# HBioquant/DiffBindFR

Hardware: AMD Instinct MI355X
Metric: poses_per_sec (higher is better)
Workload: dtype f32

## Files before the change

diffbindfr_amd/csrc/api.cpp:

```cpp
#include <cmath>
#include <cstdio>
#include <cstring>
#include <algorithm>
#include <atomic>
#include <map>

#include "launch.h"
#include "pack.h"

static unsigned long long convz_sc_lanes(const ConvZ& z) {
  unsigned long long m = 0;
  for (int i = 0; i < z.n_io; ++i) m |= 0xfffull << (z.out_off[i] / 4);
  return m;
}
static inline double fused_bytes(int D_in, int D_out) { return 4.0 * (48 + 9 + 3 + 48 + 48 + D_in + D_out); }

#define RT_TABLE static const
#include "residue_tables.inc"
#undef RT_TABLE

static thread_local std::string g_err;
void dbfr_set_error(const std::string& s) { g_err = s; }
static int fail(int code, const std::string& s) { g_err = s; return code; }

// ... 28 lines not shown
  if (!strcmp(e, "f32") || !strcmp(e, "0")) return DBFR_GEMM_F32;
  if (!strcmp(e, "split_f16") || !strcmp(e, "3")) return DBFR_GEMM_SPLIT_F16;
  if (!strcmp(e, "reduce_first") || !strcmp(e, "4")) return DBFR_GEMM_REDUCE_FIRST;
  return -1;
}

struct dbfr_model {
  dbfr_model_cfg cfg;
  std::vector<void*> allocs;
  ConvW layer[8][4];
  ConvW final_conv, tor_conv, sc_conv;
  ConvW2 layer2[8][4], tor_conv2, sc_conv2;
  ConvW2 layer2v[8][4];
  ConvZ layerz[8][4], tor_convz, sc_convz;
  int use_conv2;
  int gemm_split;
  int* queue;
  std::string fallback_convs;
  std::string rowscaled_convs;
  uint32_t layer_fallback;
  int* edge_log; int edge_log_steps, edge_log_graphs;
  int* tie_log; int tie_log_steps, tie_log_graphs; float tie_tol;
  Mlp2 lig_node_emb, lig_edge_emb, atom_edge_emb, la_edge_emb, center_edge_emb, tor_edge_emb, sc_edge_emb;
  Mlp2 tr_final, rot_final, tor_final, sc_final;
  const float* atom_emb[5]; int atom_dims[5];
  const float* atom_lin_t;
  const float *gs_lig_off, *gs_lig_c, *gs_atom_off, *gs_atom_c, *gs_cross_off, *gs_cross_c, *gs_center_off, *gs_center_c;
  int* a14_group;
  int profile;
  std::vector<hipEvent_t> ev;
// ... 182 lines not shown
      cfg->sigma_embed_dim != EMB || cfg->num_conv_layers < 1 || cfg->num_conv_layers > 8)
    return fail(DBFR_ERR_ARG, "unsupported model configuration (need ns=48, nv=12, sh_lmax=2, 32-d embeddings)");
  if (cfg->lig_edge_features + 2 * EMB > 80 || cfg->lig_node_features + EMB > 80)
    return fail(DBFR_ERR_ARG, "ligand feature width too large");
  std::string serr;
  int rc = so3_selftest(serr);
  if (rc) return fail(rc, serr);
  TMap tm;
  for (int i = 0; i < n_tensors; ++i) tm[tensors[i].name] = &tensors[i];
  dbfr_model* m = new dbfr_model();
  m->cfg = *cfg;
  m->profile = 0; m->ev_used = 0; m->flops_dev = nullptr; m->fused_bytes_last = 0; m->executed_last = 0; m->useful_last = 0; m->form_bytes_last = 0; m->conv_ms_acc = 0; m->conv_launches_acc = 0;
  m->edge_log = nullptr; m->edge_log_steps = 0; m->edge_log_graphs = 0; m->layer_fallback = 0;
  m->tie_log = nullptr; m->tie_log_steps = 0; m->tie_log_graphs = 0; m->tie_tol = 0.f;
  m->use_conv2 = getenv("DBFR_CONV2") ? atoi(getenv("DBFR_CONV2")) : -1;
  m->gemm_split = gemm_from_env();
  if (m->gemm_split < 0) rc = fail(DBFR_ERR_ARG, std::string("DBFR_GEMM=") + getenv("DBFR_GEMM") + ": unknown or retired value (f32 | split_f16 | reduce_first)");
  const char* fam[4] = {"lig_conv_layers", "cross_al_conv_layers", "atom_conv_layers", "cross_la_conv_layers"};
  for (int l = 0; l < cfg->num_conv_layers && !rc; ++l)
    for (int f = 0; f < 4 && !rc; ++f)
      rc = pack_conv144(m, tm, std::string(fam[f]) + "." + std::to_string(l), std::min(l, 3), &m->layer[l][f], &m->layer2[l][f], &m->layer2v[l][f], &m->layerz[l][f], 1u << l);
  ConvTensors final_t;
  if (!rc) rc = conv_tensors(tm, "final_conv", 4, &final_t);
  if (!rc) rc = pack_upload<PackedConv>(m, &m->final_conv, [&](PackedConv* p) { return pack_conv(final_t, 4, "final_conv", p); });
  if (!rc) rc = pack_conv144(m, tm, "tor_bond_conv", 5, &m->tor_conv, &m->tor_conv2, nullptr, &m->tor_convz, 1u << 31);
  if (!rc && !cfg->no_sc_torsion) rc = pack_conv144(m, tm, "sc_tor_bond_conv", 5, &m->sc_conv, &m->sc_conv2, nullptr, &m->sc_convz, 1u << 31);
  if (!rc) rc = pack_mlp(m, tm, "lig_node_embedding", cfg->lig_node_features + EMB, NS, NS, true, &m->lig_node_emb);
  if (!rc) rc = pack_mlp(m, tm, "lig_edge_embedding", cfg->lig_edge_features + 2 * EMB, NS, NS, true, &m->lig_edge_emb);
  if (!rc) rc = pack_mlp(m, tm, "atom_edge_embedding", 2 * EMB, NS, NS, true, &m->atom_edge_emb);
  if (!rc) rc = pack_mlp(m, tm, "la_edge_embedding", 2 * EMB, NS, NS, true, &m->la_edge_emb);
// ... 181 lines not shown
  s.chunk_es = S.chunk_es; s.chunk_gl = S.chunk_gl; s.n_chunks = S.chunk0 + G; s.max_chunks = S.chunk_cap; s.xmax = xmax; s.chunk_segs = chunk_segs;
  return s;
}

static ConvArgs conv_args(const ConvSite& s, const ConvW& cw) {
  ConvArgs a;
  a.n_edges = s.n_edges; a.max_edges = s.max_edges; a.tgt = s.tgt; a.gth = s.gth; a.emb = s.emb; a.sh = s.sh; a.sh_sign = 1.f;
  a.tab1 = s.tab1; a.ld1 = s.ld1; a.idx1 = s.idx1; a.tab2 = s.tab2; a.ld2 = s.ld2; a.idx2 = s.idx2; a.x = s.x; a.ldx = s.ldx;
  a.w = cw; a.msg = s.msg; a.trace = nullptr;
  return a;
}

static Conv2Desc conv2_desc(const ConvSite& s, const ConvW2& cw) {
  Conv2Desc d;
  d.n_edges = s.n_edges; d.max_edges = s.max_edges; d.gth = s.gth; d.emb = s.emb; d.sh = s.sh; d.tab1 = s.tab1; d.ld1 = s.ld1; d.idx1 = s.idx1;
  d.tab2 = s.tab2; d.ld2 = s.ld2; d.idx2 = s.idx2; d.x = s.x; d.ldx = s.ldx; d.w = cw; d.msg = s.msg;
  return d;
}

static ConvZDesc convz_desc(const ConvSite& s, const ConvZ& z, int D_out) {
  ConvZDesc o;
  o.n_edges = s.n_edges; o.max_edges = s.max_edges; o.tgt = s.tgt; o.gth = s.gth; o.emb = s.emb; o.sh = s.sh;
  o.tab1 = s.tab1; o.ld1 = s.ld1; o.idx1 = s.idx1; o.tab2 = s.tab2; o.ld2 = s.ld2; o.idx2 = s.idx2; o.x = s.x; o.ldx = s.ldx;
  o.w = z; o.msg = s.msg; o.D_out = D_out; o.chunk_es = s.chunk_es; o.chunk_gl = s.chunk_gl; o.n_chunks = s.n_chunks; o.max_chunks = s.max_chunks; o.xmax = s.xmax;
  return o;
}

static void conv_call(dbfr_model* m, const ConvW& cw, const ConvSite& site, hipStream_t st) {
  const ConvArgs a = conv_args(site, cw);
  hipEvent_t e0 = nullptr, e1 = nullptr;
  const bool prof = m->profile == 1 && cw.K == 144;
  const bool count = m->profile && cw.K == 144;
  if (prof) {
    prof_events(m, &e0, &e1);
    (void)hipEventRecord(e0, st);
  }
  launch_conv(a, st);
  if (prof) (void)hipEventRecord(e1, st);
  if (count) {
    launch_acc_flops(a.n_edges, 2.0 * cw.K * ((double)cw.K + cw.W), 4.0 * (cw.W + cw.D_in + 9) + 16.0, fused_bytes(cw.D_in, cw.D_out), m->flops_dev, st);
  }
}

static void conv2_call(dbfr_model* m, const Conv2Desc* descs, const int* Ws, int n, hipStream_t st, bool f16_fallback = false, const ConvZDesc* z = nullptr,
                       const int64_t* const* zsegs = nullptr) {
  Conv2Args a;
  memset(&a, 0, sizeof a);
  for (int i = 0; i < n; ++i) a.c[i] = descs[i];
  a.n_conv = n; a.queue = m->queue;
  hipEvent_t e0 = nullptr, e1 = nullptr;
  if (m->profile == 1) {
    prof_events(m, &e0, &e1);
    (void)hipEventRecord(e0, st);
  }
  static unsigned long long* trace_dev = nullptr;
  static const char* trace_file = getenv("DBFR_CONV2_TRACE");
  if (trace_file && !trace_dev) {
    if (hipMalloc(&trace_dev, 8 * C2_TRACE_CAP * sizeof(unsigned long long)) != hipSuccess) trace_dev = nullptr;
    else atexit([] {
      std::vector<unsigned long long> h(8 * C2_TRACE_CAP);
      if (hipDeviceSynchronize() == hipSuccess && hipMemcpy(h.data(), trace_dev, h.size() * 8, hipMemcpyDeviceToHost) == hipSuccess) {
        if (FILE* f = fopen(getenv("DBFR_CONV2_TRACE"), "wb")) { fwrite(h.data(), 8, h.size(), f); fclose(f); }
      }
    });
  }
  if (trace_dev) { (void)hipMemsetAsync(trace_dev, 0, 8 * C2_TRACE_CAP * sizeof(unsigned long long), st); a.trace = trace_dev; }
  if (z) {
    Conv2Args v = a;
    v.n_conv = 0;
    for (int i = 0; i < n; ++i)
      if (descs[i].w.n_tiles > 0) v.c[v.n_conv++] = descs[i];
    if (v.n_conv) launch_conv2h(v, st);
    ConvZArgs za;
    memset(&za, 0, sizeof za);
    for (int i = 0; i < n; ++i) za.c[i] = z[i];
    za.n_conv = n;
    za.dbg = nullptr;
    za.executed = m->profile ? m->flops_dev + 3 : nullptr;
    launch_convz(za, st, !zsegs);
  }
  else if (m->gemm_split >= DBFR_GEMM_SPLIT_F16 && !f16_fallback) launch_conv2h(a, st);
  else launch_conv2(a, st);
  if (m->profile == 1) (void)hipEventRecord(e1, st);
  if (m->profile) {
// ... 80 lines not shown
    const ConvSite sites[4] = {conv_site(LL, G, lx, Di, LL.tgt, lx, Di, LL.gth, lx, Di, w.msg[0], w.xmax_l, w.counters + SET_LL),
                               conv_site(AL, G, lx, Di, AL.tgt, ax, Di, AL.gth, ax, Di, w.msg[1], w.xmax_a, w.counters + SET_AL),
                               conv_site(AA, G, ax, Di, AA.tgt, ax, Di, AA.gth, ax, Di, w.msg[2], w.xmax_a, w.counters + SET_AA),
                               conv_site(LA, G, ax, Di, LA.tgt, lx, Di, LA.gth, lx, Di, w.msg[3], w.xmax_l, w.counters + SET_LA)};
    const bool fallback = (m->layer_fallback >> l) & 1u;
    const bool rf = w.conv2 && m->gemm_split == DBFR_GEMM_REDUCE_FIRST && !fallback;
    if (w.conv2) {
      Conv2Desc ds[4]; ConvZDesc zs[4]; int Ws[4]; const int64_t* sums[4];
      for (int i = 0; i < 4; ++i) {
        sums[i] = sites[i].chunk_segs;
        ds[i] = conv2_desc(sites[i], rf ? m->layer2v[l][i] : m->layer2[l][i]);
        zs[i] = convz_desc(sites[i], m->layerz[l][i], Do);
        Ws[i] = m->layer[l][i].W;
      }
      if (rf) launch_row_absmax(lx, B->lig_ptr, w.xmax_l, ax, B->atm_ptr, w.xmax_a, Di, Di, G, NA, st);
      conv2_call(m, ds, Ws, 4, st, fallback, rf ? zs : nullptr, sums);
    } else {
      ConvArgs c4[4];
      for (int i = 0; i < 4; ++i) c4[i] = conv_args(sites[i], m->layer[l][i]);
      hipEvent_t e0 = nullptr, e1 = nullptr;
      if (m->profile == 1) {
        prof_events(m, &e0, &e1);
        (void)hipEventRecord(e0, st);
      }
      launch_conv_layer(c4, st);
      if (m->profile == 1) (void)hipEventRecord(e1, st);
      if (m->profile)
        for (int i = 0; i < 4; ++i)
          launch_acc_flops(c4[i].n_edges, 2.0 * 144 * (144.0 + m->layer[l][i].W), 4.0 * (m->layer[l][i].W + Di + 9) + 16.0, fused_bytes(Di, Do), m->flops_dev, st);
    }
    ReduceLayerArgs ra;
    for (int i = 0; i < 4; ++i) {
      ra.msg[i] = sites[i].msg; ra.row_start[i] = sites[i].row_start; ra.row_cnt[i] = sites[i].row_cnt; ra.ln[i] = m->layer[l][i].ln;
      ra.first[i] = rf ? sites[i].seg_first : nullptr; ra.sc_lanes[i] = rf ? convz_sc_lanes(m->layerz[l][i]) : 0;
    }
    ra.NL = NL; ra.NA = NA; ra.D = Do; ra.D_old = Di; ra.old_l = lx; ra.old_a = ax; ra.out_l = lnew; ra.out_a = anew;
    launch_reduce_ln_layer(ra, st);
    cur ^= 1;
  }
  const int D = dims[std::min(cfg.num_conv_layers, 3)];
  if (D != MAXD) return fail(DBFR_ERR_ARG, "heads need num_conv_layers >= 3");
  const float *lx = w.lig_x[cur], *ax = w.atom_x[cur];
  launch_center_edges(*B, w.c_tgt, w.c_gth, w.c_dist, w.c_sh, w.c_row_start, w.c_row_cnt, st);
  {
    MlpArgs a; memset(&a, 0, sizeof a);
    a.w = m->center_edge_emb; a.mode = IN_TG; a.n_rows_max = NL; a.temb = w.temb; a.row_graph_tab = w.lig_batch;
    a.dist = w.c_dist; a.gs_offset = m->gs_center_off; a.gs_coeff = m->gs_center_c; a.out = w.c_emb;
    launch_mlp(a, st);
  }
  conv_call(m, m->final_conv, flat_site(w.n_edges6 + 7, NL, w.c_tgt, w.c_gth, w.c_emb, w.c_sh, lx, D, w.c_gth, nullptr, 0, w.c_gth, lx, D, w.msg[0]), st);
  launch_reduce_ln(w.msg[0], w.c_row_start, w.c_row_cnt, G, 12, m->final_conv.ln, nullptr, 0, w.gp, 12, 2, st);
// ... 467 lines not shown
}

extern "C" int dbfr_test_reduce_ln_layer(const dbfr_model* m, int32_t layer, const float* const* msg, const int32_t* const* row_start,
                                         const int32_t* const* row_cnt, const uint8_t* const* seg_first, int32_t NL, int32_t NA, const float* old_l,
                                         const float* old_a, float* out_l, float* out_a, void* hip_stream) {
  if (!m || !msg || !row_start || !row_cnt || !old_l || !old_a || !out_l || !out_a) return fail(DBFR_ERR_ARG, "dbfr_test_reduce_ln_layer: null argument");
  if (layer < 0 || layer >= m->cfg.num_conv_layers || NL < 0 || NA < 0) return fail(DBFR_ERR_ARG, "dbfr_test_reduce_ln_layer: no such layer");
  ReduceLayerArgs ra;
  for (int i = 0; i < 4; ++i) {
    if (!msg[i] || !row_start[i] || !row_cnt[i] || (seg_first && !seg_first[i])) return fail(DBFR_ERR_ARG, "dbfr_test_reduce_ln_layer: null edge-set argument");
    ra.msg[i] = msg[i]; ra.row_start[i] = row_start[i]; ra.row_cnt[i] = row_cnt[i]; ra.ln[i] = m->layer[layer][i].ln;
    ra.first[i] = seg_first ? seg_first[i] : nullptr; ra.sc_lanes[i] = seg_first ? convz_sc_lanes(m->layerz[layer][i]) : 0;
  }
  ra.NL = NL; ra.NA = NA; ra.D = m->layer[layer][0].D_out; ra.D_old = m->layer[layer][0].D_in;
  ra.old_l = old_l; ra.old_a = old_a; ra.out_l = out_l; ra.out_a = out_a;
  launch_reduce_ln_layer(ra, (hipStream_t)hip_stream);
  HIPCHECK(hipGetLastError());
  return DBFR_OK;
}

extern "C" int dbfr_test_center_edges(const dbfr_batch* b, int32_t* tgt, int32_t* gth, float* dist, float* sh, int32_t* row_start, int32_t* row_cnt,
                                      void* hip_stream) {
  if (!b || !tgt || !gth || !dist || !sh || !row_start || !row_cnt || !b->lig_ptr || !b->lig_pos || b->G <= 0)
    return fail(DBFR_ERR_ARG, "dbfr_test_center_edges: null argument");
  launch_center_edges(*b, tgt, gth, dist, sh, row_start, row_cnt, (hipStream_t)hip_stream);
  HIPCHECK(hipGetLastError());
  return DBFR_OK;
}

extern "C" int dbfr_test_trrot(const dbfr_model* m, const float* gp, const float* temb, const float* tr_sigma, const float* rot_norm, int32_t G,
// ... 31 lines not shown
```

diffbindfr_amd/csrc/common.h:

```cpp
#pragma once
#include <hip/hip_runtime.h>
#include <stdint.h>
#include <string.h>
#include <string>
#include <vector>

#include "../../include/dbfr.h"

#define NS 48
#define NV 12
#define SH_LD 9
#define EMB 32
#define MAXD 168
#define EDGE_CHUNK 64
int dbfr_edge_chunks(int max_na, int max_nl);

typedef float f32x4 __attribute__((ext_vector_type(4)));
typedef float f32x2 __attribute__((ext_vector_type(2)));
typedef _Float16 f16x8 __attribute__((ext_vector_type(8)));
typedef _Float16 f16x4 __attribute__((ext_vector_type(4)));
typedef _Float16 f16x2 __attribute__((ext_vector_type(2)));
typedef unsigned u32x4 __attribute__((ext_vector_type(4)));
typedef unsigned u32x2 __attribute__((ext_vector_type(2)));

// ... 63 lines not shown
  const void* W2h;
  const RunDesc* runs;
  int part_run[4][9];
};

struct Conv2Desc {
  const int* n_edges; int max_edges;
  const int* gth;
  const float* emb;
  const float* sh;
  const float* tab1; int ld1; const int* idx1;
  const float* tab2; int ld2; const int* idx2;
  const float* x; int ldx;
  ConvW2 w;
  float* msg;
};

struct Conv2Args {
  Conv2Desc c[4];
  int n_conv;
  int* queue;
  int run_barrier, no_split;
  int skew;
  unsigned long long* trace;
};
#define C2_TRACE_CAP 4096

#define CZ_NKT 10
#define CZ_MAXCT 12
#define CZ_MAXSEG 4
#define CZ_TILE_BYTES 6144
struct ConvZ {
  int n_io;
  int nct[2];
  int ct0[2];
  int out_off[2];
  int nc_valid[2];
  const uint32_t* cdesc;
// ... 95 lines not shown
```

diffbindfr_amd/csrc/conv.hip:

```cpp
#include <cstdio>
#include <cstdlib>
#include <type_traits>
#include <vector>

#include "launch.h"

#ifndef CONV_PRIO
#define CONV_PRIO 0
#endif
#ifndef CONV_XPF
#define CONV_XPF 0
#endif
#ifndef CONV_NB2_WAVES
#define CONV_NB2_WAVES 2
#endif
#define XS_LD (MAXD + 4)

#define TRACE_BLOCKS 1024
#define TRACE_TILES 48
#define TRACE_REC (2 + 3 * TRACE_TILES + 8)
#define RSTAMP(k) do { if ((ABL & 16) && a.trace && bid < TRACE_BLOCKS && lane == 0) a.trace[((size_t)bid * 4 + wave) * TRACE_REC + 2 + 3 * TRACE_TILES + (k)] = __builtin_amdgcn_s_memrealtime(); } while (0)
#define TSTAMP(k) do { if ((ABL & 16) && a.trace && bid < TRACE_BLOCKS && lane == 0) a.trace[((size_t)bid * 4 + wave) * TRACE_REC + 2 + 3 * TRACE_TILES + (k)] = __builtin_readcyclecounter(); } while (0)

template <int K, int NB, int ABL>
// ... 383 lines not shown
      (void)hipFree(d);
      if (FILE* f = fopen(trace_path, "wb")) { fwrite(h.data(), 8, nw, f); fclose(f); }
      trace_path = nullptr;
      return;
    }
  }
#define LAUNCH(KK, AB) hipLaunchKernelGGL((k_conv<KK, CONV_NB, AB>), dim3(tiles), dim3(256), 0, st, b)
  if (a.w.K != 144) { LAUNCH(96, 0); return; }
#ifdef DBFR_DEV_VARIANTS
  switch (abl) { case 1: LAUNCH(144, 1); return; case 2: LAUNCH(144, 2); return; case 8: LAUNCH(144, 8); return; default: break; }
#endif
  LAUNCH(144, 0);
#undef LAUNCH
}

__device__ __forceinline__ f32x4 row_sum(const float* __restrict__ msg, int rs, int rc, int D, int lane, const uint8_t* __restrict__ first, unsigned long long sc_lanes) {
  const int d4 = D >> 2;
  f32x4 acc = {0.f, 0.f, 0.f, 0.f};
  const f32x4* r = reinterpret_cast<const f32x4*>(msg + (size_t)rs * D) + min(lane, d4 - 1);
  if (!first) {
    if (lane < d4) {
      int e = 0;
      for (; e + 8 <= rc; e += 8) {
        const f32x4 v0 = r[(size_t)e * d4], v1 = r[(size_t)(e + 1) * d4], v2 = r[(size_t)(e + 2) * d4], v3 = r[(size_t)(e + 3) * d4];
        const f32x4 v4 = r[(size_t)(e + 4) * d4], v5 = r[(size_t)(e + 5) * d4], v6 = r[(size_t)(e + 6) * d4], v7 = r[(size_t)(e + 7) * d4];
        acc += v0; acc += v1; acc += v2; acc += v3; acc += v4; acc += v5; acc += v6; acc += v7;
      }
      for (; e + 4 <= rc; e += 4) {
        const f32x4 v0 = r[(size_t)e * d4], v1 = r[(size_t)(e + 1) * d4], v2 = r[(size_t)(e + 2) * d4], v3 = r[(size_t)(e + 3) * d4];
        acc += v0; acc += v1; acc += v2; acc += v3;
      }
      for (; e < rc; ++e) acc += r[(size_t)e * d4];
    }
    return acc;
  }
  const bool sc = (sc_lanes >> lane) & 1ull;
  const f32x4 zero = {0.f, 0.f, 0.f, 0.f};
  for (int e0 = 0; e0 < rc; e0 += 64) {
    const int nb = min(64, rc - e0);
    const unsigned long long fl = __ballot(lane < nb && first[rs + e0 + lane] != 0);
    if (lane < d4) {
      int e = 0;
      auto row = [&](int i) { return (!sc || ((fl >> i) & 1ull)) ? r[(size_t)(e0 + i) * d4] : zero; };
      for (; e + 8 <= nb; e += 8) {
        const f32x4 v0 = row(e), v1 = row(e + 1), v2 = row(e + 2), v3 = row(e + 3), v4 = row(e + 4), v5 = row(e + 5), v6 = row(e + 6), v7 = row(e + 7);
        acc += v0; acc += v1; acc += v2; acc += v3; acc += v4; acc += v5; acc += v6; acc += v7;
      }
      for (; e + 4 <= nb; e += 4) {
        const f32x4 v0 = row(e), v1 = row(e + 1), v2 = row(e + 2), v3 = row(e + 3);
        acc += v0; acc += v1; acc += v2; acc += v3;
      }
      for (; e < nb; ++e)
        if (!sc || ((fl >> e) & 1ull)) acc += r[(size_t)(e0 + e) * d4];
    }
  }
  return acc;
}

__global__ __launch_bounds__(256) void k_reduce_ln(const float* __restrict__ msg, const int* __restrict__ row_start,
                                                   const int* __restrict__ row_cnt, int N, int D, LNDesc ln,
                                                   const float* __restrict__ old, int D_old, float* __restrict__ out,
                                                   int ldo, int mode, const uint8_t* first, unsigned long long sc_lanes) {
  __shared__ float buf[4][MAXD];
  const int lane = threadIdx.x & 63, wave = threadIdx.x >> 6;
  const int node_raw = blockIdx.x * 4 + wave;
  const bool live = node_raw < N;
  const int node = live ? node_raw : N - 1;
  const int rs = row_start[node], rc = row_cnt[node];
  const int d4 = D >> 2;
  const f32x4 acc = row_sum(msg, rs, rc, D, lane, first, sc_lanes);
  if (lane < d4) {
    const float cntf = (float)max(rc, 1);
    float* bw = buf[wave] + 4 * lane;
    bw[0] = acc[0] / cntf; bw[1] = acc[1] / cntf; bw[2] = acc[2] / cntf; bw[3] = acc[3] / cntf;
  }
  __syncthreads();
  int iw = 0, ib = 0;
  for (int bk = 0; bk < ln.nblk; ++bk) {
    const int mul = ln.mul[bk], dim = ln.dim[bk], off = ln.off[bk];
    const int nel = mul * dim;
    float mean[3] = {0.f, 0.f, 0.f};
    for (int i = lane; i < nel; i += 64) {
      int comp = i % dim;
      float v = buf[wave][off + i];
      if (comp == 0) mean[0] += v; else if (comp == 1) mean[1] += v; else mean[2] += v;
// ... 25 lines not shown
  __syncthreads();
#pragma unroll
  for (int j = 0; j < 3; ++j) {
    int c = lane + 64 * j;
    if (c < D && live) {
      float v = buf[wave][c];
      float* o = out + (size_t)node * ldo + c;
      if (mode == 0) v = (c < D_old ? old[(size_t)node * D_old + c] : 0.f) + v;
      else if (mode == 1) v = *o + v;
      *o = v;
    }
  }
}

void launch_reduce_ln(const float* msg, const int* row_start, const int* row_cnt, int N, int D, const LNDesc& ln,
                      const float* old, int D_old, float* out, int ldo, int mode, hipStream_t st, const uint8_t* first, unsigned long long sc_lanes) {
  if (N <= 0) return;
  hipLaunchKernelGGL(k_reduce_ln, dim3((N + 3) / 4), dim3(256), 0, st, msg, row_start, row_cnt, N, D, ln, old, D_old,
                     out, ldo, mode, first, sc_lanes);
}

__device__ __forceinline__ void mean_ln(const float* __restrict__ msg, int rs, int rc, int D, const LNDesc& ln, float* bw, int lane, const uint8_t* first, unsigned long long sc_lanes) {
  const int d4 = D >> 2;
  const f32x4 acc = row_sum(msg, rs, rc, D, lane, first, sc_lanes);
  if (lane < d4) {
    const float cntf = (float)max(rc, 1);
    bw[4 * lane] = acc[0] / cntf; bw[4 * lane + 1] = acc[1] / cntf; bw[4 * lane + 2] = acc[2] / cntf; bw[4 * lane + 3] = acc[3] / cntf;
  }
  __builtin_amdgcn_wave_barrier();
  int iw = 0, ib = 0;
  for (int bk = 0; bk < ln.nblk; ++bk) {
    const int mul = ln.mul[bk], dim = ln.dim[bk], off = ln.off[bk];
    const int nel = mul * dim;
    float mean[3] = {0.f, 0.f, 0.f};
    const bool d3 = dim == 3;
    for (int i = lane; i < nel; i += 64) {
      int comp = d3 ? i % 3 : 0;
      float v = bw[off + i];
      if (comp == 0) mean[0] += v; else if (comp == 1) mean[1] += v; else mean[2] += v;
// ... 17 lines not shown
    __builtin_amdgcn_wave_barrier();
    for (int o = 32; o > 0; o >>= 1) sq += __shfl_xor(sq, o);
    const float inv = 1.0f / sqrtf(sq / (float)nel + 1e-5f);
    for (int i = lane; i < nel; i += 64) {
      int u = d3 ? i / 3 : i;
      float v = bw[off + i] * (inv * ln.weight[iw + u]);
      if (ln.is0e[bk]) v += ln.bias[ib + u];
      bw[off + i] = v;
    }
    iw += mul;
    if (ln.is0e[bk]) ib += mul;
  }
  __builtin_amdgcn_wave_barrier();
}

__global__ __launch_bounds__(256) void k_reduce_ln_layer(ReduceLayerArgs a) {
  __shared__ float buf[4][2][MAXD];
  const int lane = threadIdx.x & 63, wave = threadIdx.x >> 6;
  const int nbl = (a.NL + 3) / 4;
  const bool lig = (int)blockIdx.x < nbl;
  const int node = (lig ? blockIdx.x : blockIdx.x - nbl) * 4 + wave;
  const int N = lig ? a.NL : a.NA;
  if (node >= N) return;
  const int s0 = lig ? 0 : 2;
  mean_ln(a.msg[s0], a.row_start[s0][node], a.row_cnt[s0][node], a.D, a.ln[s0], buf[wave][0], lane, a.first[s0], a.sc_lanes[s0]);
  mean_ln(a.msg[s0 + 1], a.row_start[s0 + 1][node], a.row_cnt[s0 + 1][node], a.D, a.ln[s0 + 1], buf[wave][1], lane, a.first[s0 + 1], a.sc_lanes[s0 + 1]);
  const float* old = (lig ? a.old_l : a.old_a) + (size_t)node * a.D_old;
  float* out = (lig ? a.out_l : a.out_a) + (size_t)node * a.D;
#pragma unroll
  for (int j = 0; j < 3; ++j) {
    const int c = lane + 64 * j;
    if (c < a.D) out[c] = ((c < a.D_old ? old[c] : 0.f) + buf[wave][0][c]) + buf[wave][1][c];
  }
}

template <int O> __device__ __forceinline__ float xor_lane(float x) {
  if constexpr (O == 8) return __int_as_float(__builtin_amdgcn_update_dpp(0, __float_as_int(x), 0x128, 0xf, 0xf, false));
  else if constexpr (O == 2) return __int_as_float(__builtin_amdgcn_update_dpp(0, __float_as_int(x), 0x4e, 0xf, 0xf, false));
  else if constexpr (O == 1) return __int_as_float(__builtin_amdgcn_update_dpp(0, __float_as_int(x), 0xb1, 0xf, 0xf, false));
  else return __shfl_xor(x, O);
}

template <int O, int N> __device__ __forceinline__ void xor_stage(float (&x)[N]) {
  float y[N];
#pragma unroll
  for (int i = 0; i < N; ++i) y[i] = xor_lane<O>(x[i]);
#pragma unroll
  for (int i = 0; i < N; ++i) x[i] += y[i];
}

template <int N> __device__ __forceinline__ void xor_butterflies(float (&x)[N]) {
  xor_stage<32>(x); xor_stage<16>(x); xor_stage<8>(x); xor_stage<4>(x); xor_stage<2>(x); xor_stage<1>(x);
}

template <int NBLK>
__global__ __launch_bounds__(256, NBLK == 4 ? 7 : 8) void k_reduce_ln_layer_fixed(ReduceLayerArgs a) {
  constexpr int D = NBLK == 2 ? 84 : NBLK == 3 ? 120 : MAXD;
  constexpr int MUL[4] = {48, 12, 12, 48}, DIM[4] = {1, 3, 3, 1}, OFF[4] = {0, 48, 84, 120}, IW[4] = {0, 48, 60, 72};
  constexpr int NCH = NBLK == 2 ? 4 : NBLK == 3 ? 7 : 8;
  __shared__ float buf[4][2][MAXD];
  const int lane = threadIdx.x & 63, wave = threadIdx.x >> 6;
  const int nbl = (a.NL + 3) / 4;
  const bool lig = (int)blockIdx.x < nbl;
  const int node = (lig ? blockIdx.x : blockIdx.x - nbl) * 4 + wave;
  const int N = lig ? a.NL : a.NA;
  if (node >= N) return;
  const int s0 = lig ? 0 : 2;
  const int rs0 = a.row_start[s0][node], rc0 = a.row_cnt[s0][node], rs1 = a.row_start[s0 + 1][node], rc1 = a.row_cnt[s0 + 1][node];
  f32x4 acc[2];
  acc[0] = row_sum(a.msg[s0], rs0, rc0, D, lane, a.first[s0], a.sc_lanes[s0]);
  acc[1] = row_sum(a.msg[s0 + 1], rs1, rc1, D, lane, a.first[s0 + 1], a.sc_lanes[s0 + 1]);
  const float* old = (lig ? a.old_l : a.old_a) + (size_t)node * a.D_old;
  float shift[2][NBLK], weight[2][NBLK], bias[2], oldv[NBLK];
  unsigned el[NBLK];
#pragma unroll
  for (int b = 0; b < NBLK; ++b) {
    el[b] = min(lane, MUL[b] * DIM[b] - 1);
    const unsigned un = IW[b] + (DIM[b] == 3 ? el[b] / 3u : el[b]);
#pragma unroll
    for (int s = 0; s < 2; ++s) { shift[s][b] = a.ln[s0 + s].mean_shift[un]; weight[s][b] = a.ln[s0 + s].weight[un]; }
    oldv[b] = OFF[b] + el[b] < (unsigned)a.D_old ? old[OFF[b] + el[b]] : 0.f;
  }
#pragma unroll
  for (int s = 0; s < 2; ++s) bias[s] = a.ln[s0 + s].bias[el[0]];
  if (lane < D / 4) {
#pragma unroll
// ... 52 lines not shown
static int reduce_ln_fixed_layout(const ReduceLayerArgs& a) {
  static const int mul[4] = {48, 12, 12, 48}, dim[4] = {1, 3, 3, 1}, off[4] = {0, 48, 84, 120};
  const int nblk = a.ln[0].nblk;
  if (nblk < 2 || nblk > 4 || a.D != off[nblk - 1] + mul[nblk - 1] * dim[nblk - 1] || a.D_old > a.D) return 0;
  for (int s = 0; s < 4; ++s) {
    if (a.ln[s].nblk != nblk) return 0;
    for (int b = 0; b < nblk; ++b)
      if (a.ln[s].mul[b] != mul[b] || a.ln[s].dim[b] != dim[b] || a.ln[s].off[b] != off[b] || (a.ln[s].is0e[b] != 0) != (b == 0)) return 0;
  }
  return nblk;
}

void launch_reduce_ln_layer(const ReduceLayerArgs& a, hipStream_t st) {
  const int nb = (a.NL + 3) / 4 + (a.NA + 3) / 4;
  if (nb <= 0) return;
  switch (reduce_ln_fixed_layout(a)) {
    case 2: hipLaunchKernelGGL(k_reduce_ln_layer_fixed<2>, dim3(nb), dim3(256), 0, st, a); break;
    case 3: hipLaunchKernelGGL(k_reduce_ln_layer_fixed<3>, dim3(nb), dim3(256), 0, st, a); break;
    case 4: hipLaunchKernelGGL(k_reduce_ln_layer_fixed<4>, dim3(nb), dim3(256), 0, st, a); break;
    default: hipLaunchKernelGGL(k_reduce_ln_layer, dim3(nb), dim3(256), 0, st, a);
  }
}
```

diffbindfr_amd/csrc/conv2h.hip:

```cpp
#include <cstdio>
#include <cstdlib>
#include <type_traits>

#include "launch.h"

#define CH_TILE_BYTES 9280
#define CH_TAIL_OFF 8192
#define CH_BIAS_OFF 9216
#define CH_RING_BYTES 10240

__device__ __forceinline__ void split2x2(float x0, float x1, unsigned& hi, unsigned& lo) {
  const f16x2 h = __builtin_convertvector((f32x2){x0, x1}, f16x2);
  const f16x2 l = __builtin_convertvector((f32x2){x0 - (float)h[0], x1 - (float)h[1]}, f16x2);
  hi = __builtin_bit_cast(unsigned, h);
  lo = __builtin_bit_cast(unsigned, l);
}

__device__ __forceinline__ void scale4(f32x4& o, const f32x4& v, float s) { o[0] = v[0] * s; o[1] = v[1] * s; o[2] = v[2] * s; o[3] = v[3] * s; }
__device__ __forceinline__ void sum4(f32x4& o, const f32x4& a, const f32x4& b) { o[0] = a[0] + b[0]; o[1] = a[1] + b[1]; o[2] = a[2] + b[2]; o[3] = a[3] + b[3]; }

#define C2_XLD 124
#define C2_WAVE_FLOATS (32 * C2_XLD + 32 * 10 + 32 * 8 + 32)

template <int NW, int ABL = 0>
__global__ __launch_bounds__(64 * NW, 2) void k_conv2h(Conv2Args a) {
  constexpr int K = 144, KT = 9;
  constexpr bool ROWF = (ABL & 1024) != 0;
  constexpr int EPB = 32 * NW;
  extern __shared__ __attribute__((aligned(16))) float lds[];
  const int tid = threadIdx.x, lane = tid & 63, wave = tid >> 6;
  const int n = lane & 15, g = lane >> 4;
  if (wave >= NW / 2) __builtin_amdgcn_s_setprio(1);
  const char* ring = reinterpret_cast<const char*>(lds);
  float* xs = lds + CH_RING_BYTES / 4 + wave * C2_WAVE_FLOATS;
  float* shs = xs + 32 * C2_XLD;
  float* ms = shs + 32 * 10;
  int* s_gth = reinterpret_cast<int*>(ms + 32 * 8);

  if (a.trace && blockIdx.x == 0 && tid == 0) { a.trace[0] = __builtin_readcyclecounter(); a.trace[1] = __builtin_amdgcn_s_memrealtime(); }
// ... 47 lines not shown
    char* ringw = const_cast<char*>(ring);
    u32x4 stgA = {0u, 0u, 0u, 0u};
    u32x2 stgB = {0u, 0u};
    auto fetchA = [&](int tile) { if (!(ABL & (4 | 16))) stgA = __builtin_bit_cast(u32x4, __builtin_amdgcn_raw_buffer_load_b128(rW, vA, ((ABL & 512) ? (tile & 7) : tile) * CH_TILE_BYTES + offA, 0)); };
    auto fetchB = [&](int tile) { if (!(ABL & (4 | 16))) stgB = __builtin_bit_cast(u32x2, __builtin_amdgcn_raw_buffer_load_b64(rW, lane * 8, ((ABL & 512) ? (tile & 7) : tile) * CH_TILE_BYTES + offB, 0)); };
    auto putA = [&] { if (!(ABL & (4 | 8))) *reinterpret_cast<u32x4*>(ringw + offA + vW) = stgA; };
    auto putB = [&] { if (!(ABL & (4 | 8))) *reinterpret_cast<u32x2*>(ringw + offB + lane * 8) = stgB; };
    using I0 = std::integral_constant<int, 0>; using I1 = std::integral_constant<int, 1>;
    using I2 = std::integral_constant<int, 2>; using I3 = std::integral_constant<int, 3>;
    if (r_begin < r_end) {
      fetchA(t_first); fetchB(t_first);
    }

    int ev[2], gthv[2];
    const float* r0[2]; const float* r1[2]; const float* r2[2];
#pragma unroll
    for (int b = 0; b < 2; ++b) {
      const int e = e0 + 16 * b + n;
      ev[b] = min(e, E - 1);
      gthv[b] = d.gth[ev[b]];
      r0[b] = d.emb + (size_t)ev[b] * NS;
      r1[b] = d.tab1 + (size_t)d.idx1[ev[b]] * d.ld1;
      r2[b] = d.tab2 + (size_t)d.idx2[ev[b]] * d.ld2;
    }
    if (g == 0) { s_gth[n] = gthv[0]; s_gth[16 + n] = gthv[1]; }
    if (lane < 32) {
      const int e = min(e0 + lane, E - 1);
      const float* sp = d.sh + (size_t)e * SH_LD;
      float s[9];
#pragma unroll
      for (int k = 0; k < 9; ++k) { s[k] = sp[k]; shs[lane * 10 + k] = s[k]; }
      const float r3 = 1.7320508075688772f;
      float* m = ms + lane * 8;
      m[0] = -s[6] - r3 * s[8]; m[1] = r3 * s[5]; m[2] = r3 * s[4]; m[3] = 2.f * s[6]; m[4] = r3 * s[7]; m[5] = -s[6] + r3 * s[8];
    }
    u32x4 Bh[2][2][4];
    u32x4 Btc[2];
    float se[2], ue[2];
    {
      const __amdgpu_buffer_rsrc_t rW1 = __builtin_amdgcn_make_buffer_rsrc((void*)d.w.W1h, 0, KT * CH_TILE_BYTES, 0x00020000);
      u32x4 Ah[2][2][4];
      u32x4 Atc[2];
      float sa[2];
      int ja[2];
#pragma unroll
      for (int b = 0; b < 2; ++b) {
        f32x4 Ba[KT];
        float amx = 0.f;
#pragma unroll
// ... 304 lines not shown
        const float* xp = xs_lane + xo;
        accp[0] = (f32x4){0.f, 0.f, 0.f, 0.f}; accp[1] = (f32x4){0.f, 0.f, 0.f, 0.f};
        for (int i = 0; i < nt; ++i) {
          tile(tile0 + i, [&](auto mc) { travel(mc, xp); });
          if (i) xp += x_step;
        }
        __builtin_amdgcn_sched_barrier(0);
#define COPS(b) cop(b, std::integral_constant<int, 0>{}, xp); cop(b, std::integral_constant<int, 1>{}, xp); cop(b, std::integral_constant<int, 2>{}, xp); \
        cop(b, std::integral_constant<int, 3>{}, xp); cop(b, std::integral_constant<int, 4>{}, xp); cop(b, std::integral_constant<int, 5>{}, xp); \
        cop(b, std::integral_constant<int, 6>{}, xp); cop(b, std::integral_constant<int, 7>{}, xp); cop(b, std::integral_constant<int, 8>{}, xp); \
        cop(b, std::integral_constant<int, 9>{}, xp); cop(b, std::integral_constant<int, 10>{}, xp); cop(b, std::integral_constant<int, 11>{}, xp); \
        cop(b, std::integral_constant<int, 12>{}, xp); finish(b);
        COPS(B0{}) COPS(B1{})
#undef COPS
        if (flags & 2) {
          if (oo < D_out) {
#pragma unroll
            for (int b = 0; b < 2; ++b)
              if (e0 + 16 * b + n < E) {
                float* op = d.msg + (size_t)(e0 + 16 * b + n) * D_out + oo;
                op[0] = oacc[b][0] * ue[b];
                if (VOUT) { op[1] = oacc[b][1] * ue[b]; op[2] = oacc[b][2] * ue[b]; }
              }
          }
        }
      };
      switch (type) {
        case PT_SS: run(std::integral_constant<int, PT_SS>{}); break;
        case PT_SV: run(std::integral_constant<int, PT_SV>{}); break;
        case PT_VS: run(std::integral_constant<int, PT_VS>{}); break;
        case PT_VVS: run(std::integral_constant<int, PT_VVS>{}); break;
// ... 14 lines not shown
  static int no_split = getenv("DBFR_CONV2_NOSPLIT") ? atoi(getenv("DBFR_CONV2_NOSPLIT")) : 0;
  constexpr int NW = 8;
  const size_t lds = CH_RING_BYTES + (size_t)NW * C2_WAVE_FLOATS * sizeof(float);
  const int n_cu = dbfr_current_cu_count();
  Conv2Args b = a;
  b.skew = 0;
  b.run_barrier = 0;
  b.no_split = no_split;
#define V(x) { if (dbfr_launch_check(hipFuncSetAttribute(reinterpret_cast<const void*>(&k_conv2h<NW, x>), hipFuncAttributeMaxDynamicSharedMemorySize, (int)lds), "k_conv2h: hipFuncSetAttribute(MaxDynamicSharedMemorySize)")) return; \
               hipLaunchKernelGGL((k_conv2h<NW, x>), dim3(n_cu), dim3(64 * NW), lds, st, b); return; }
#ifdef DBFR_DEV_VARIANTS
  static int abl = getenv("DBFR_CONV2H_ABL") ? atoi(getenv("DBFR_CONV2H_ABL")) : 0;
  if (abl == 1) V(1) if (abl == 2) V(2) if (abl == 3) V(3) if (abl == 4) V(4) if (abl == 7) V(7) if (abl == 8) V(8) if (abl == 16) V(16)
  if (abl == 32) V(32) if (abl == 64) V(64) if (abl == 256) V(256) if (abl == 512) V(512)
#endif
  for (int i = 0; i < a.n_conv; ++i)
    if (a.c[i].w.W2rinv || a.c[i].w.W1rinv) V(1024)
  V(0)
#undef V
}
```

diffbindfr_amd/csrc/launch.h:

```cpp
#pragma once
#include "common.h"

#define MAX_NL 256
#define MAX_NA 8192

void launch_conv(const ConvArgs& a, hipStream_t st);
void launch_conv_layer(const ConvArgs* c4, hipStream_t st);
void launch_conv2(const Conv2Args& a, hipStream_t st);
void launch_conv2h(const Conv2Args& a, hipStream_t st);
void launch_convz(const ConvZArgs& a, hipStream_t st, bool useful_pass = false);
void launch_reduce_ln(const float* msg, const int* row_start, const int* row_cnt, int N, int D, const LNDesc& ln,
                      const float* old, int D_old, float* out, int ldo, int mode, hipStream_t st, const uint8_t* first = nullptr, unsigned long long sc_lanes = 0);
struct ReduceLayerArgs {
  const float* msg[4]; const int* row_start[4]; const int* row_cnt[4]; LNDesc ln[4];
  int NL, NA, D, D_old;
  const float* old_l; const float* old_a; float* out_l; float* out_a;
  const uint8_t* first[4]; unsigned long long sc_lanes[4];
};
void launch_reduce_ln_layer(const ReduceLayerArgs& a, hipStream_t st);

enum SetKind { SET_LL = 0, SET_AA = 1, SET_AL = 2, SET_LA = 3, SET_TOR = 4, SET_SC = 5, N_SETS = 6 };

struct GraphArgs {
  dbfr_batch b;
  const int* lig_batch;
  const int* atm_batch;
  const uint8_t* is_cab;
  const int* n_cab;
  const float* tr_sigma;
  float lig_cut2, atom_cut2, cross_cut2;
  int lig_cap, atom_cap, dynamic_cross;
  EdgeSet set[N_SETS];
// ... 86 lines not shown
```

Baseline: 546.6.

## Fold per-target vector message runs in conv2h epilogue before scatter

Adds a FOLD variant of the conv2h kernel. It detects segment boundaries from target indices, builds a wave-level open mask, and sums consecutive edges with the same target using DPP row shifts, storing only one partial per run within each 32-edge tile. The reduce/LayerNorm kernels get a matching VEC_FOLDED template that reads only run-start rows (plus the first partial row) for vector lanes. The aim is to cut message stores and reduction reads. In exchange it adds DPP shift loops, extra tgt loads and more kernel instantiations, and it depends on edges being sorted by target.

```diff
diff --git a/diffbindfr_amd/csrc/api.cpp b/diffbindfr_amd/csrc/api.cpp
--- a/diffbindfr_amd/csrc/api.cpp
+++ b/diffbindfr_amd/csrc/api.cpp
@@ -66,6 +66,7 @@
   ConvW2 layer2v[8][4];
   ConvZ layerz[8][4], tor_convz, sc_convz;
   int use_conv2;
+  int vec_fold;
   int gemm_split;
   int* queue;
   std::string fallback_convs;
@@ -278,6 +279,7 @@
   m->edge_log = nullptr; m->edge_log_steps = 0; m->edge_log_graphs = 0; m->layer_fallback = 0;
   m->tie_log = nullptr; m->tie_log_steps = 0; m->tie_log_graphs = 0; m->tie_tol = 0.f;
   m->use_conv2 = getenv("DBFR_CONV2") ? atoi(getenv("DBFR_CONV2")) : -1;
+  m->vec_fold = getenv("DBFR_VEC_FOLD") ? atoi(getenv("DBFR_VEC_FOLD")) != 0 : 1;
   m->gemm_split = gemm_from_env();
   if (m->gemm_split < 0) rc = fail(DBFR_ERR_ARG, std::string("DBFR_GEMM=") + getenv("DBFR_GEMM") + ": unknown or retired value (f32 | split_f16 | reduce_first)");
   const char* fam[4] = {"lig_conv_layers", "cross_al_conv_layers", "atom_conv_layers", "cross_la_conv_layers"};
@@ -489,7 +491,7 @@
 static Conv2Desc conv2_desc(const ConvSite& s, const ConvW2& cw) {
   Conv2Desc d;
   d.n_edges = s.n_edges; d.max_edges = s.max_edges; d.gth = s.gth; d.emb = s.emb; d.sh = s.sh; d.tab1 = s.tab1; d.ld1 = s.ld1; d.idx1 = s.idx1;
-  d.tab2 = s.tab2; d.ld2 = s.ld2; d.idx2 = s.idx2; d.x = s.x; d.ldx = s.ldx; d.w = cw; d.msg = s.msg;
+  d.tab2 = s.tab2; d.ld2 = s.ld2; d.idx2 = s.idx2; d.x = s.x; d.ldx = s.ldx; d.w = cw; d.msg = s.msg; d.tgt = s.tgt;
   return d;
 }
 
@@ -518,7 +520,7 @@
 }
 
 static void conv2_call(dbfr_model* m, const Conv2Desc* descs, const int* Ws, int n, hipStream_t st, bool f16_fallback = false, const ConvZDesc* z = nullptr,
-                       const int64_t* const* zsegs = nullptr) {
+                       const int64_t* const* zsegs = nullptr, bool fold = false) {
   Conv2Args a;
   memset(&a, 0, sizeof a);
   for (int i = 0; i < n; ++i) a.c[i] = descs[i];
@@ -543,6 +545,7 @@
   if (z) {
     Conv2Args v = a;
     v.n_conv = 0;
+    v.fold = fold;
     for (int i = 0; i < n; ++i)
       if (descs[i].w.n_tiles > 0) v.c[v.n_conv++] = descs[i];
     if (v.n_conv) launch_conv2h(v, st);
@@ -653,7 +656,7 @@
         Ws[i] = m->layer[l][i].W;
       }
       if (rf) launch_row_absmax(lx, B->lig_ptr, w.xmax_l, ax, B->atm_ptr, w.xmax_a, Di, Di, G, NA, st);
-      conv2_call(m, ds, Ws, 4, st, fallback, rf ? zs : nullptr, sums);
+      conv2_call(m, ds, Ws, 4, st, fallback, rf ? zs : nullptr, sums, rf && m->vec_fold);
     } else {
       ConvArgs c4[4];
       for (int i = 0; i < 4; ++i) c4[i] = conv_args(sites[i], m->layer[l][i]);
@@ -674,6 +677,7 @@
       ra.first[i] = rf ? sites[i].seg_first : nullptr; ra.sc_lanes[i] = rf ? convz_sc_lanes(m->layerz[l][i]) : 0;
     }
     ra.NL = NL; ra.NA = NA; ra.D = Do; ra.D_old = Di; ra.old_l = lx; ra.old_a = ax; ra.out_l = lnew; ra.out_a = anew;
+    ra.vec_folded = rf && m->vec_fold;
     launch_reduce_ln_layer(ra, st);
     cur ^= 1;
   }
@@ -1171,6 +1175,7 @@
   }
   ra.NL = NL; ra.NA = NA; ra.D = m->layer[layer][0].D_out; ra.D_old = m->layer[layer][0].D_in;
   ra.old_l = old_l; ra.old_a = old_a; ra.out_l = out_l; ra.out_a = out_a;
+  ra.vec_folded = 0;
   launch_reduce_ln_layer(ra, (hipStream_t)hip_stream);
   HIPCHECK(hipGetLastError());
   return DBFR_OK;
diff --git a/diffbindfr_amd/csrc/common.h b/diffbindfr_amd/csrc/common.h
--- a/diffbindfr_amd/csrc/common.h
+++ b/diffbindfr_amd/csrc/common.h
@@ -101,6 +101,7 @@
   const float* x; int ldx;
   ConvW2 w;
   float* msg;
+  const int* tgt;
 };
 
 struct Conv2Args {
@@ -109,6 +110,7 @@
   int* queue;
   int run_barrier, no_split;
   int skew;
+  int fold;
   unsigned long long* trace;
 };
 #define C2_TRACE_CAP 4096
diff --git a/diffbindfr_amd/csrc/conv.hip b/diffbindfr_amd/csrc/conv.hip
--- a/diffbindfr_amd/csrc/conv.hip
+++ b/diffbindfr_amd/csrc/conv.hip
@@ -421,6 +421,7 @@
 #undef LAUNCH
 }
 
+template <bool VEC_FOLDED>
 __device__ __forceinline__ f32x4 row_sum(const float* __restrict__ msg, int rs, int rc, int D, int lane, const uint8_t* __restrict__ first, unsigned long long sc_lanes) {
   const int d4 = D >> 2;
   f32x4 acc = {0.f, 0.f, 0.f, 0.f};
@@ -443,12 +444,36 @@
   }
   const bool sc = (sc_lanes >> lane) & 1ull;
   const f32x4 zero = {0.f, 0.f, 0.f, 0.f};
+  if constexpr (!VEC_FOLDED) {
+    for (int e0 = 0; e0 < rc; e0 += 64) {
+      const int nb = min(64, rc - e0);
+      const unsigned long long fl = __ballot(lane < nb && first[rs + e0 + lane] != 0);
+      if (lane < d4) {
+        int e = 0;
+        auto row = [&](int i) { return (!sc || ((fl >> i) & 1ull)) ? r[(size_t)(e0 + i) * d4] : zero; };
+        for (; e + 8 <= nb; e += 8) {
+          const f32x4 v0 = row(e), v1 = row(e + 1), v2 = row(e + 2), v3 = row(e + 3), v4 = row(e + 4), v5 = row(e + 5), v6 = row(e + 6), v7 = row(e + 7);
+          acc += v0; acc += v1; acc += v2; acc += v3; acc += v4; acc += v5; acc += v6; acc += v7;
+        }
+        for (; e + 4 <= nb; e += 4) {
+          const f32x4 v0 = row(e), v1 = row(e + 1), v2 = row(e + 2), v3 = row(e + 3);
+          acc += v0; acc += v1; acc += v2; acc += v3;
+        }
+        for (; e < nb; ++e)
+          if (!sc || ((fl >> e) & 1ull)) acc += r[(size_t)(e0 + e) * d4];
+      }
+    }
+    return acc;
+  }
+  const int raw0 = min(rc, 32 - (rs & 31));
   for (int e0 = 0; e0 < rc; e0 += 64) {
     const int nb = min(64, rc - e0);
     const unsigned long long fl = __ballot(lane < nb && first[rs + e0 + lane] != 0);
+    const unsigned long long vl = e0 ? ~0ull : (~0ull << raw0) | 1ull;
     if (lane < d4) {
       int e = 0;
-      auto row = [&](int i) { return (!sc || ((fl >> i) & 1ull)) ? r[(size_t)(e0 + i) * d4] : zero; };
+      auto have = [&](int i) { const bool f = (fl >> i) & 1ull, v = (vl >> i) & 1ull; return sc ? f : v; };
+      auto row = [&](int i) { return have(i) ? r[(size_t)(e0 + i) * d4] : zero; };
       for (; e + 8 <= nb; e += 8) {
         const f32x4 v0 = row(e), v1 = row(e + 1), v2 = row(e + 2), v3 = row(e + 3), v4 = row(e + 4), v5 = row(e + 5), v6 = row(e + 6), v7 = row(e + 7);
         acc += v0; acc += v1; acc += v2; acc += v3; acc += v4; acc += v5; acc += v6; acc += v7;
@@ -458,12 +483,13 @@
         acc += v0; acc += v1; acc += v2; acc += v3;
       }
       for (; e < nb; ++e)
-        if (!sc || ((fl >> e) & 1ull)) acc += r[(size_t)(e0 + e) * d4];
+        if (have(e)) acc += r[(size_t)(e0 + e) * d4];
     }
   }
   return acc;
 }
 
+template <bool VEC_FOLDED>
 __global__ __launch_bounds__(256) void k_reduce_ln(const float* __restrict__ msg, const int* __restrict__ row_start,
                                                    const int* __restrict__ row_cnt, int N, int D, LNDesc ln,
                                                    const float* __restrict__ old, int D_old, float* __restrict__ out,
@@ -475,7 +501,7 @@
   const int node = live ? node_raw : N - 1;
   const int rs = row_start[node], rc = row_cnt[node];
   const int d4 = D >> 2;
-  const f32x4 acc = row_sum(msg, rs, rc, D, lane, first, sc_lanes);
+  const f32x4 acc = row_sum<VEC_FOLDED>(msg, rs, rc, D, lane, first, sc_lanes);
   if (lane < d4) {
     const float cntf = (float)max(rc, 1);
     float* bw = buf[wave] + 4 * lane;
@@ -531,15 +557,17 @@
 }
 
 void launch_reduce_ln(const float* msg, const int* row_start, const int* row_cnt, int N, int D, const LNDesc& ln,
-                      const float* old, int D_old, float* out, int ldo, int mode, hipStream_t st, const uint8_t* first, unsigned long long sc_lanes) {
+                      const float* old, int D_old, float* out, int ldo, int mode, hipStream_t st, const uint8_t* first, unsigned long long sc_lanes, bool vec_folded) {
   if (N <= 0) return;
-  hipLaunchKernelGGL(k_reduce_ln, dim3((N + 3) / 4), dim3(256), 0, st, msg, row_start, row_cnt, N, D, ln, old, D_old,
-                     out, ldo, mode, first, sc_lanes);
-}
-
+  if (vec_folded && first) hipLaunchKernelGGL(k_reduce_ln<true>, dim3((N + 3) / 4), dim3(256), 0, st, msg, row_start, row_cnt, N, D, ln, old, D_old, out, ldo, mode, first, sc_lanes);
+  else hipLaunchKernelGGL(k_reduce_ln<false>, dim3((N + 3) / 4), dim3(256), 0, st, msg, row_start, row_cnt, N, D, ln, old, D_old,
+                          out, ldo, mode, first, sc_lanes);
+}
+
+template <bool VEC_FOLDED>
 __device__ __forceinline__ void mean_ln(const float* __restrict__ msg, int rs, int rc, int D, const LNDesc& ln, float* bw, int lane, const uint8_t* first, unsigned long long sc_lanes) {
   const int d4 = D >> 2;
-  const f32x4 acc = row_sum(msg, rs, rc, D, lane, first, sc_lanes);
+  const f32x4 acc = row_sum<VEC_FOLDED>(msg, rs, rc, D, lane, first, sc_lanes);
   if (lane < d4) {
     const float cntf = (float)max(rc, 1);
     bw[4 * lane] = acc[0] / cntf; bw[4 * lane + 1] = acc[1] / cntf; bw[4 * lane + 2] = acc[2] / cntf; bw[4 * lane + 3] = acc[3] / cntf;
@@ -587,6 +615,7 @@
   __builtin_amdgcn_wave_barrier();
 }
 
+template <bool VEC_FOLDED>
 __global__ __launch_bounds__(256) void k_reduce_ln_layer(ReduceLayerArgs a) {
   __shared__ float buf[4][2][MAXD];
   const int lane = threadIdx.x & 63, wave = threadIdx.x >> 6;
@@ -596,8 +625,8 @@
   const int N = lig ? a.NL : a.NA;
   if (node >= N) return;
   const int s0 = lig ? 0 : 2;
-  mean_ln(a.msg[s0], a.row_start[s0][node], a.row_cnt[s0][node], a.D, a.ln[s0], buf[wave][0], lane, a.first[s0], a.sc_lanes[s0]);
-  mean_ln(a.msg[s0 + 1], a.row_start[s0 + 1][node], a.row_cnt[s0 + 1][node], a.D, a.ln[s0 + 1], buf[wave][1], lane, a.first[s0 + 1], a.sc_lanes[s0 + 1]);
+  mean_ln<VEC_FOLDED>(a.msg[s0], a.row_start[s0][node], a.row_cnt[s0][node], a.D, a.ln[s0], buf[wave][0], lane, a.first[s0], a.sc_lanes[s0]);
+  mean_ln<VEC_FOLDED>(a.msg[s0 + 1], a.row_start[s0 + 1][node], a.row_cnt[s0 + 1][node], a.D, a.ln[s0 + 1], buf[wave][1], lane, a.first[s0 + 1], a.sc_lanes[s0 + 1]);
   const float* old = (lig ? a.old_l : a.old_a) + (size_t)node * a.D_old;
   float* out = (lig ? a.out_l : a.out_a) + (size_t)node * a.D;
 #pragma unroll
@@ -626,7 +655,7 @@
   xor_stage<32>(x); xor_stage<16>(x); xor_stage<8>(x); xor_stage<4>(x); xor_stage<2>(x); xor_stage<1>(x);
 }
 
-template <int NBLK>
+template <int NBLK, bool VEC_FOLDED>
 __global__ __launch_bounds__(256, NBLK == 4 ? 7 : 8) void k_reduce_ln_layer_fixed(ReduceLayerArgs a) {
   constexpr int D = NBLK == 2 ? 84 : NBLK == 3 ? 120 : MAXD;
   constexpr int MUL[4] = {48, 12, 12, 48}, DIM[4] = {1, 3, 3, 1}, OFF[4] = {0, 48, 84, 120}, IW[4] = {0, 48, 60, 72};
@@ -641,8 +670,8 @@
   const int s0 = lig ? 0 : 2;
   const int rs0 = a.row_start[s0][node], rc0 = a.row_cnt[s0][node], rs1 = a.row_start[s0 + 1][node], rc1 = a.row_cnt[s0 + 1][node];
   f32x4 acc[2];
-  acc[0] = row_sum(a.msg[s0], rs0, rc0, D, lane, a.first[s0], a.sc_lanes[s0]);
-  acc[1] = row_sum(a.msg[s0 + 1], rs1, rc1, D, lane, a.first[s0 + 1], a.sc_lanes[s0 + 1]);
+  acc[0] = row_sum<VEC_FOLDED>(a.msg[s0], rs0, rc0, D, lane, a.first[s0], a.sc_lanes[s0]);
+  acc[1] = row_sum<VEC_FOLDED>(a.msg[s0 + 1], rs1, rc1, D, lane, a.first[s0 + 1], a.sc_lanes[s0 + 1]);
   const float* old = (lig ? a.old_l : a.old_a) + (size_t)node * a.D_old;
   float shift[2][NBLK], weight[2][NBLK], bias[2], oldv[NBLK];
   unsigned el[NBLK];
@@ -725,10 +754,13 @@
 void launch_reduce_ln_layer(const ReduceLayerArgs& a, hipStream_t st) {
   const int nb = (a.NL + 3) / 4 + (a.NA + 3) / 4;
   if (nb <= 0) return;
+  const bool vf = a.vec_folded && a.first[0] && a.first[1] && a.first[2] && a.first[3];
+#define GO(...) { if (vf) hipLaunchKernelGGL((__VA_ARGS__ true>), dim3(nb), dim3(256), 0, st, a); else hipLaunchKernelGGL((__VA_ARGS__ false>), dim3(nb), dim3(256), 0, st, a); }
   switch (reduce_ln_fixed_layout(a)) {
-    case 2: hipLaunchKernelGGL(k_reduce_ln_layer_fixed<2>, dim3(nb), dim3(256), 0, st, a); break;
-    case 3: hipLaunchKernelGGL(k_reduce_ln_layer_fixed<3>, dim3(nb), dim3(256), 0, st, a); break;
-    case 4: hipLaunchKernelGGL(k_reduce_ln_layer_fixed<4>, dim3(nb), dim3(256), 0, st, a); break;
-    default: hipLaunchKernelGGL(k_reduce_ln_layer, dim3(nb), dim3(256), 0, st, a);
-  }
-}
+    case 2: GO(k_reduce_ln_layer_fixed<2,) break;
+    case 3: GO(k_reduce_ln_layer_fixed<3,) break;
+    case 4: GO(k_reduce_ln_layer_fixed<4,) break;
+    default: GO(k_reduce_ln_layer<)
+  }
+#undef GO
+}
diff --git a/diffbindfr_amd/csrc/conv2h.hip b/diffbindfr_amd/csrc/conv2h.hip
--- a/diffbindfr_amd/csrc/conv2h.hip
+++ b/diffbindfr_amd/csrc/conv2h.hip
@@ -19,10 +19,51 @@
 __device__ __forceinline__ void scale4(f32x4& o, const f32x4& v, float s) { o[0] = v[0] * s; o[1] = v[1] * s; o[2] = v[2] * s; o[3] = v[3] * s; }
 __device__ __forceinline__ void sum4(f32x4& o, const f32x4& a, const f32x4& b) { o[0] = a[0] + b[0]; o[1] = a[1] + b[1]; o[2] = a[2] + b[2]; o[3] = a[3] + b[3]; }
 
+__device__ __forceinline__ float row_shr1(float x) { return __int_as_float(__builtin_amdgcn_update_dpp(0, __float_as_int(x), 0x111, 0xf, 0xf, true)); }
+__device__ __forceinline__ float row_ror1(float x) { return __int_as_float(__builtin_amdgcn_update_dpp(0, __float_as_int(x), 0x121, 0xf, 0xf, false)); }
+template <int NC>
+__device__ __forceinline__ void fold_runs(float (&v)[2][3], unsigned open_v, int ne, int n, bool (&store)[2], int (&row)[2]) {
+  const unsigned open = __builtin_amdgcn_readfirstlane(open_v);
+  const int first = open ? __builtin_ctz(open) : 32;
+  const unsigned long long stop = (unsigned long long)open | (1ull << ne);
+  bool cont[2];
+  float p[2][NC];
+#pragma unroll
+  for (int b = 0; b < 2; ++b) {
+    const int i = 16 * b + n;
+    const bool opens = (open >> i) & 1u;
+    cont[b] = i > first && !opens && i < ne;
+    store[b] = i < ne && (i < first || ((stop >> (i + 1)) & 1ull));
+    row[b] = i < first ? i : 31 - __clz((int)(open & (0xffffffffu >> (31 - i))));
+#pragma unroll
+    for (int k = 0; k < NC; ++k) p[b][k] = opens ? 0.f + v[b][k] : v[b][k];
+  }
+  const unsigned conts = ~open & (first < 31 ? ~((2u << first) - 1u) : 0u) & (ne < 32 ? (1u << ne) - 1u : ~0u);
+  auto longest = [](unsigned x) { int l = 0; while (x) { x &= x >> 1; ++l; } return l; };
+  const int steps0 = longest(conts & 0xffffu), steps1 = longest(conts >> 16);
+  for (int s = 0; s < steps0; s += 4)
+#pragma unroll
+    for (int u = 0; u < 4; ++u)
+#pragma unroll
+      for (int k = 0; k < NC; ++k) { const float t = row_shr1(p[0][k]) + v[0][k]; p[0][k] = cont[0] ? t : p[0][k]; }
+  const bool c0 = cont[1] && n == 0, c1 = cont[1] && n != 0;
+#pragma unroll
+  for (int k = 0; k < NC; ++k) { const float t = row_ror1(p[0][k]) + v[1][k]; p[1][k] = c0 ? t : p[1][k]; }
+  for (int s = 0; s < steps1; s += 4)
+#pragma unroll
+    for (int u = 0; u < 4; ++u)
+#pragma unroll
+      for (int k = 0; k < NC; ++k) { const float t = row_shr1(p[1][k]) + v[1][k]; p[1][k] = c1 ? t : p[1][k]; }
+#pragma unroll
+  for (int b = 0; b < 2; ++b)
+#pragma unroll
+    for (int k = 0; k < NC; ++k) v[b][k] = p[b][k];
+}
+
 #define C2_XLD 124
 #define C2_WAVE_FLOATS (32 * C2_XLD + 32 * 10 + 32 * 8 + 32)
 
-template <int NW, int ABL = 0>
+template <int NW, int ABL = 0, bool FOLD = false>
 __global__ __launch_bounds__(64 * NW, 2) void k_conv2h(Conv2Args a) {
   constexpr int K = 144, KT = 9;
   constexpr bool ROWF = (ABL & 1024) != 0;
@@ -100,16 +141,23 @@
 
     int ev[2], gthv[2];
     const float* r0[2]; const float* r1[2]; const float* r2[2];
+    bool opens[2] = {false, false};
 #pragma unroll
     for (int b = 0; b < 2; ++b) {
       const int e = e0 + 16 * b + n;
       ev[b] = min(e, E - 1);
       gthv[b] = d.gth[ev[b]];
+      if constexpr (FOLD) {
+        const int t_me = d.tgt[ev[b]], t_prev = d.tgt[max(ev[b] - 1, 0)];
+        opens[b] = e < E && (e == 0 || t_me != t_prev);
+      }
       r0[b] = d.emb + (size_t)ev[b] * NS;
       r1[b] = d.tab1 + (size_t)d.idx1[ev[b]] * d.ld1;
       r2[b] = d.tab2 + (size_t)d.idx2[ev[b]] * d.ld2;
     }
     if (g == 0) { s_gth[n] = gthv[0]; s_gth[16 + n] = gthv[1]; }
+    unsigned seg_open = 0;
+    if constexpr (FOLD) seg_open = ((unsigned)__ballot(opens[0]) & 0xffffu) | ((unsigned)__ballot(opens[1]) << 16);
     if (lane < 32) {
       const int e = min(e0 + lane, E - 1);
       const float* sp = d.sh + (size_t)e * SH_LD;
@@ -119,6 +167,7 @@
       const float r3 = 1.7320508075688772f;
       float* m = ms + lane * 8;
       m[0] = -s[6] - r3 * s[8]; m[1] = r3 * s[5]; m[2] = r3 * s[4]; m[3] = 2.f * s[6]; m[4] = r3 * s[7]; m[5] = -s[6] + r3 * s[8];
+      if constexpr (FOLD) m[6] = __uint_as_float(seg_open);
     }
     u32x4 Bh[2][2][4];
     u32x4 Btc[2];
@@ -453,7 +502,28 @@
         COPS(B0{}) COPS(B1{})
 #undef COPS
         if (flags & 2) {
-          if (oo < D_out) {
+          if constexpr (FOLD) {
+            float val[2][3];
+            bool store[2];
+            int row[2];
+#pragma unroll
+            for (int b = 0; b < 2; ++b)
+#pragma unroll
+              for (int k = 0; k < 3; ++k) {
+                val[b][k] = oacc[b][k] * ue[b];
+                asm volatile("" : "+v"(val[b][k]));
+              }
+            fold_runs<VOUT ? 3 : 1>(val, __float_as_uint(ms[n * 8 + 6]), min(max(E - e0, 0), 32), n, store, row);
+            if (oo < D_out) {
+#pragma unroll
+              for (int b = 0; b < 2; ++b)
+                if (store[b]) {
+                  float* op = d.msg + (size_t)(e0 + row[b]) * D_out + oo;
+                  op[0] = val[b][0];
+                  if (VOUT) { op[1] = val[b][1]; op[2] = val[b][2]; }
+                }
+            }
+          } else if (oo < D_out) {
 #pragma unroll
             for (int b = 0; b < 2; ++b)
               if (e0 + 16 * b + n < E) {
@@ -498,8 +568,12 @@
   if (abl == 1) V(1) if (abl == 2) V(2) if (abl == 3) V(3) if (abl == 4) V(4) if (abl == 7) V(7) if (abl == 8) V(8) if (abl == 16) V(16)
   if (abl == 32) V(32) if (abl == 64) V(64) if (abl == 256) V(256) if (abl == 512) V(512)
 #endif
+#define VF(x) { if (dbfr_launch_check(hipFuncSetAttribute(reinterpret_cast<const void*>(&k_conv2h<NW, x, true>), hipFuncAttributeMaxDynamicSharedMemorySize, (int)lds), "k_conv2h: hipFuncSetAttribute(MaxDynamicSharedMemorySize)")) return; \
+                hipLaunchKernelGGL((k_conv2h<NW, x, true>), dim3(n_cu), dim3(64 * NW), lds, st, b); return; }
   for (int i = 0; i < a.n_conv; ++i)
-    if (a.c[i].w.W2rinv || a.c[i].w.W1rinv) V(1024)
+    if (a.c[i].w.W2rinv || a.c[i].w.W1rinv) { if (a.fold) VF(1024) else V(1024) }
+  if (a.fold) VF(0)
   V(0)
+#undef VF
 #undef V
 }
diff --git a/diffbindfr_amd/csrc/launch.h b/diffbindfr_amd/csrc/launch.h
--- a/diffbindfr_amd/csrc/launch.h
+++ b/diffbindfr_amd/csrc/launch.h
@@ -10,12 +10,14 @@
 void launch_conv2h(const Conv2Args& a, hipStream_t st);
 void launch_convz(const ConvZArgs& a, hipStream_t st, bool useful_pass = false);
 void launch_reduce_ln(const float* msg, const int* row_start, const int* row_cnt, int N, int D, const LNDesc& ln,
-                      const float* old, int D_old, float* out, int ldo, int mode, hipStream_t st, const uint8_t* first = nullptr, unsigned long long sc_lanes = 0);
+                      const float* old, int D_old, float* out, int ldo, int mode, hipStream_t st, const uint8_t* first = nullptr, unsigned long long sc_lanes = 0,
+                      bool vec_folded = false);
 struct ReduceLayerArgs {
   const float* msg[4]; const int* row_start[4]; const int* row_cnt[4]; LNDesc ln[4];
   int NL, NA, D, D_old;
   const float* old_l; const float* old_a; float* out_l; float* out_a;
   const uint8_t* first[4]; unsigned long long sc_lanes[4];
+  int vec_folded;
 };
 void launch_reduce_ln_layer(const ReduceLayerArgs& a, hipStream_t st);
 
```

Measured after the change: 544.9. About the same (-0.3%).
